# bark-simulator/planner-miqp

Hardware: AMD Instinct MI355X
Metric: MIQP solves/sec to 1% gap, 2-agent x 20-step x 32-region (higher is better)
Workload: dtype f64

## Files before the change

### planner_miqp_amd/csrc/as_onchip.hip

```cpp
namespace miqp {

#ifdef MIQP_PROFILE
#define ASP_T(var) const long long var = clock64()
#define ASP_ACC(k, t0, t1) asp_[k] += (unsigned long long)((t1) - (t0))
#else
#define ASP_T(var)
#define ASP_ACC(k, t0, t1)
#endif
constexpr int AS_MAXSTEP = 220;
constexpr double AS_VTOL = 1.0e-8;
constexpr double AS_DEP = 1.0e-8;
constexpr int AS_MT = 64;
constexpr int AS_MSTR = AS_MT * (AS_MT + 1) / 2;

__host__ __device__ constexpr bool as_shape_ok(int C, int N) { return (C == 1 || C == 2) && N >= 1 && N <= 2 * OC_NSL; }

template <int C> __device__ inline int as_col(int pq) { return C == 2 ? ((pq & 3) << 2) | (pq >> 2) : ((pq & 1) << 2) | (pq >> 1); }
template <int C> __device__ inline int as_pcol(int q) { return C == 2 ? ((q & 3) << 2) | (q >> 2) : ((q & 3) << 1) | (q >> 2); }

template <int C, int NSL, int GCAP = miqp::OC_GCAP>
__global__ void __launch_bounds__(64, (GCAP > 128 ? 1 : 2)) as_onchip_kernel(DevBuf B) {
  static_assert(C == 1 || C == 2, "a stage of 16 columns holds the chains of up to two cars");
  constexpr bool CM = true;
  constexpr bool BIG = GCAP > 128;
  constexpr int OC_GCAP = GCAP, OC_GSLOTS = OC_GCAP / 64, OC_GCOEF = oc_gcoef_of(OC_GCAP);
  constexpr int NX = 6 * C, NZ = 8 * C, NCH = 2 * C;
  const Layout& Y = B.Y;
  const int tid = threadIdx.x, lg = tid >> 4, lc = tid & 15;
  const int par = lg >> 1, side = lg & 1;
  const double bsgn = side ? -1.0 : 1.0;
  WAVE_DUMP(BIG ? 1 : 4);
  const int* const clist = BIG && B.cls_take ? B.cls_list + (size_t)(B.cls_take - 1) * B.batch_cap : nullptr;
  const int nbatch = clist ? (B.cls_count[B.cls_take - 1] < B.batch_cap ? B.cls_count[B.cls_take - 1] : B.batch_cap) : (*B.batch_count < B.batch_cap ? *B.batch_count : B.batch_cap);
  const int N = Y.N, NSLOT = Y.NSLOT;
  extern __shared__ double lds[];
  char* const L0 = (char*)lds;
  const OcLds LL = oc_lds_layout(N, Y.fixlen, OC_GCAP, !BIG);
  double* const Z = (double*)(L0 + LL.z);
  double* const scr = (double*)(L0 + LL.u);
  double* const V = (double*)(L0 + LL.u);
  unsigned long long* const bkey = (unsigned long long*)(L0 + LL.r);
  const int SPAN = LL.gmeta - LL.u;
  double* const kref = (double*)(L0 + LL.u + SPAN - N * 32);
  double* const kff = kref - N * 4;
  double* const KS = kff - N * 16;
  const int STG_CAP = (SPAN - N * 192) / 8;
  uint4* const gmeta = (uint4*)(L0 + LL.gmeta);
  double* const gcoef = (double*)(L0 + LL.gcoef);
  double* const grhs = (double*)(L0 + LL.grhs);
  double* const Wd = (double*)(L0 + LL.wd);
  int* const sstart = (int*)(L0 + LL.sstart);
  unsigned short* const cand = (unsigned short*)(L0 + LL.cand);
// ... 6 lines not shown
  const int chunk = B.as_chunk > 0 ? B.as_chunk : 1;
  int run_next = 0, run_end = 0;
  const int quota = BIG ? 0 : B.as_quota; int handed = 0;
#ifdef MIQP_PROFILE
  const unsigned long long wv_c0 = __builtin_amdgcn_s_memtime(), wv_r0 = __builtin_amdgcn_s_memrealtime();
  unsigned long long wv_first = 0; int wv_nodes = 0;
  if (!BIG && tid == 0) wv_first = atomicMin(&B.prof[120], wv_r0);
#endif
  for (;;) {
    __syncthreads();
    if (run_next >= run_end) {
      if (quota > 0 && handed >= quota) break;
      ++handed;
      if (tid == 0) sh_node = atomicAdd(B.work_counter, chunk);
      __syncthreads();
      run_next = __builtin_amdgcn_readfirstlane(sh_node); run_end = run_next + chunk;
      if (run_next >= nbatch) break;
    }
    const int slot_ = run_next++;
    if (slot_ >= nbatch) { run_next = run_end; continue; }
    const int node = clist ? __builtin_amdgcn_readfirstlane(clist[slot_]) : slot_;
    {
      const int cls = B.batch_large ? (int)B.batch_large[node] : (is_probe_word(B.batch_depth[node]) ? 1 : 0);
      if (cls != (BIG ? 1 : 0)) continue;
    }
    WAVE_DUMP_NODE();
    const int inst = __builtin_amdgcn_readfirstlane(B.batch_inst[node]);
    const double* D = B.inst_d + (size_t)inst * Y.dstride;
    const int* T = B.inst_i + (size_t)inst * Y.istride;
    const double ts = D[Y.d_glob + 7];
    const double aqs = 2.0 * D[Y.d_misc + 0];
    const double iaq = aqs > 0.0 ? 1.0 / aqs : 0.0;
    {
      const signed char* src = B.pool_fix + (size_t)B.batch_node[node] * Y.fixlen;
      for (int k = tid; k < Y.fixlen; k += 64) fix[k] = src[k];
      if (tid < 16) Wd[tid] = tid < NZ ? D[Y.d_wd + oc_lcol<C, CM>(as_pcol<C>(tid))] : 0.0;
      for (int k = tid; k < N * 32; k += 64) bkey[k] = ~0ull;
      for (int k = tid; k <= N + 1; k += 64) sstart[k] = 0;
    }
    __syncthreads();
    const double* Rf = D + Y.d_ref;
    double cutoff = 1e300;
    {
      const double inc0 = fmin(inc_from_key(*(volatile unsigned long long*)&B.inc_key[inst]), B.inc_ext[inst]);
      const double gap_ = is_probe_word(B.batch_depth[node]) ? 0.0 : B.inst_gap[inst];
      if (B.use_cutoff && inc0 < 1e300) cutoff = inc0 - gap_ * (1e-10 + fabs(inc0)) - B.inst_const[inst];
    }

#ifdef MIQP_PROFILE
    unsigned long long asp_[12] = {0, 0, 0, 0, 0, 0, 0, 0, 0, 0, 0, 0};
#endif
    ASP_T(ta0);
    int ngen = 0;
    {
      unsigned long long* const bmp = (unsigned long long*)scr;
      const int nw = (N * NSLOT + 63) >> 6;
      unsigned short* const pre = (unsigned short*)(bmp + nw);
      for (int k = tid; k < nw; k += 64) bmp[k] = 0ull;
      OC_WAVE_SYNC();
      const int cls_off[8] = {0, 7, 11, 16, 16 + Y.EL, 16 + 5 * Y.EL, C * Y.SC, C * Y.SC + 8 * Y.NP};
      const int cls_cnt[8] = {7, 4, 5, Y.EL, 4 * Y.EL, 5 * Y.O, 8 * Y.NP, 16 * Y.NP};
      auto take = [&](int i, int slot) {
        if (decode_row<C, false>(Y, D, T, fix, i, slot, nullptr).active) {
          int col; double sg, rh;
          if (box_of_slot<C>(Y, D, T, fix, i, slot, col, sg, rh)) atomicMin(&bkey[(i * 2 + (sg < 0.0 ? 1 : 0)) * 16 + as_col<C>(oc_pcol<C, CM>(col))], d2key(rh));
          else { const int pcode = i * NSLOT + slot; atomicOr(&bmp[pcode >> 6], 1ull << (pcode & 63)); }
        }
      };
      unsigned short* const plist = pre + ((nw + 1 + 3) & ~3);
      const int LCAP = (int)(((char*)(L0 + LL.r) - (char*)plist) / 2) - 64;
      int nlist = 0;
      auto flush = [&]() {
        OC_WAVE_SYNC();
        for (int j0 = 0; j0 < nlist; j0 += 64) if (j0 + tid < nlist) { const int pc = plist[j0 + tid]; const int i = pc / NSLOT; take(i, pc - i * NSLOT); }
        OC_WAVE_SYNC();
        nlist = 0;
      };
      for (int e0 = 0; e0 < C * N; e0 += 64) {
        const int e = e0 + tid;
        if (e < C * N) {
          const int c = e / N, i = e - c * N;
          const double* G = D + Y.d_glob;
          const int code = i >= 1 ? (int)fix[Y.f_reg + c * N + i] : -1;
          const unsigned int skip = i >= 1 ? (unsigned int)T[Y.i_boxskip + c * N + i] : 0x7Fu;
          const double* rt = code >= 0 ? D + Y.d_reg + (c * Y.P + (code >> 2)) * REGSZ : nullptr;
          const double* Hc = (!rt && i >= 1) ? region_hull(Y, D, T, fix, c, i) : nullptr;
          auto put = [&](int col, bool neg, double rh) { atomicMin(&bkey[(i * 2 + (neg ? 1 : 0)) * 16 + as_col<C>(oc_pcol<C, CM>(col))], d2key(rh)); };
          if (i >= 1) {
            const double a_lo_x = rt ? rt[11] : Hc[0], a_hi_x = rt ? rt[12] : Hc[1], a_lo_y = rt ? rt[13] : Hc[2], a_hi_y = rt ? rt[14] : Hc[3];
            if (!(skip & 1u)) put(6 * c + 1, true, -G[0]);
            if (!(skip & 2u)) put(6 * c + 4, true, -G[0]);
            if (!(skip & 4u)) put(6 * c + 1, false, G[1]);
            if (!(skip & 8u)) put(6 * c + 2, false, a_hi_x);
            if (!(skip & 16u)) put(6 * c + 2, true, -a_lo_x);
            if (!(skip & 32u)) put(6 * c + 5, false, a_hi_y);
            if (!(skip & 64u)) put(6 * c + 5, true, -a_lo_y);
          }
          if (i <= N - 2) {
#pragma unroll
            for (int s_ = 0; s_ < 2; ++s_) {
              double lo, hi;
              if (i == 0) { lo = D[Y.d_u0box + c * 4 + 2 * s_]; hi = D[Y.d_u0box + c * 4 + 2 * s_ + 1]; }
              else if (rt) { lo = rt[15 + 2 * s_]; hi = rt[16 + 2 * s_]; }
              else { lo = Hc[4 + 2 * s_]; hi = Hc[5 + 2 * s_]; }
              put(6 * C + 2 * c + s_, false, hi); put(6 * C + 2 * c + s_, true, -lo);
            }
          }
        }
      }
#pragma unroll 1
      for (int cl = 0; cl < 8; ++cl) {
#ifdef MIQP_PROFILE
        if (cl == 2) { const long long tq_ = clock64(); asp_[9] += (unsigned long long)(tq_ - ta0); }
#endif
        const int cnt = cls_cnt[cl], off = cls_off[cl];
        const bool percar = cl < 6;
        const int per = percar ? C * cnt : cnt, total = N * per;
        for (int e0 = 0; e0 < total; e0 += 64) {
          const int e = e0 + tid;
          int i = 0, slot = 0; bool in = e < total;
          if (in) { i = e / per; const int rem = e - i * per; slot = percar ? (rem / cnt) * Y.SC + off + rem % cnt : off + rem; }
          if (cl < 2) continue;
          const bool cnd = in && slot_maybe<C>(Y, fix, i, slot);
          const unsigned long long mk = __ballot(cnd);
          if (cnd) plist[nlist + __popcll(mk & lt)] = (unsigned short)(i * NSLOT + slot);
          nlist += __popcll(mk);
          if (nlist > LCAP) flush();
        }
      }
      flush();
      if (tid == 0) { int a = 0; for (int k = 0; k < nw; ++k) { pre[k] = (unsigned short)(a < 65535 ? a : 65535); a += __popcll(bmp[k]); } pre[nw] = (unsigned short)(a < 65535 ? a : 65535); }
      OC_WAVE_SYNC();
      ngen = pre[nw];
      if (ngen <= OC_GCAP)
        for (int k = tid; k < nw; k += 64) {
          unsigned long long bits = bmp[k]; int pos = pre[k];
          while (bits) { const int b = __ffsll((long long)bits) - 1; cand[pos++] = (unsigned short)(k * 64 + b); bits &= bits - 1ull; }
        }
      OC_WAVE_SYNC();
    }
#ifdef MIQP_PROFILE
    const long long tq1_ = clock64();
#endif
    bool overflow = ngen > OC_GCAP;
    int ncoef = 0;
    for (int c0 = 0; c0 < ngen && !overflow; c0 += OC_SCR) {
      double* g = scr + (tid & (OC_SCR - 1)) * OC_SSTR;
      RowOut r; r.active = false; r.rhs = 0; r.aq = 0;
      int i = 0, nn = 0;
      const bool mine = tid < OC_SCR && c0 + tid < ngen;
      int slot_ = 0;
      if (mine) { const int pcode = cand[c0 + tid]; i = pcode / NSLOT; slot_ = pcode - i * NSLOT; r = decode_row<C, true>(Y, D, T, fix, i, slot_, g); }
      unsigned long long map = 0ull; unsigned int cols = 0u;
      double v6[6];
#pragma unroll
      for (int k = 0; k < 6; ++k) v6[k] = 0.0;
      if (mine) {
        for (int q = 0; q < NZ; ++q) {
          const double v = g[q];
          if (v != 0.0 && nn < 6) {
#pragma unroll
            for (int k = 0; k < 6; ++k) if (k == nn) v6[k] = v;
            const int pq = as_col<C>(oc_pcol<C, CM>(q));
            map |= (unsigned long long)(nn + 1) << (4 * pq); cols |= (unsigned int)pq << (4 * nn); nn++;
          }
        }
      }
      const bool keep = mine && nn > 0;
      const unsigned long long mk = __ballot(keep);
      const unsigned long long b0 = __ballot(keep && (nn & 1)), b1 = __ballot(keep && (nn & 2)), b2 = __ballot(keep && (nn & 4));
      const int tot = __popcll(b0) + 2 * __popcll(b1) + 4 * __popcll(b2);
      if (ncoef + tot > OC_GCOEF) { overflow = true; break; }
      if (keep) {
        const int idx = sstart[N + 1] + __popcll(mk & lt);
        const int off = ncoef + __popcll(b0 & lt) + 2 * __popcll(b1 & lt) + 4 * __popcll(b2 & lt);
#pragma unroll
        for (int k = 0; k < 6; ++k) if (k < nn) gcoef[off + k] = v6[k];
        uint4 m4; m4.x = (unsigned int)map; m4.y = (unsigned int)(map >> 32);
        m4.z = (unsigned int)off | ((unsigned int)nn << 16) | ((unsigned int)i << 20) | (r.aq > 0.0 ? 0x80000000u : 0u); m4.w = cols;
        gmeta[idx] = m4; grhs[idx] = r.rhs;
        cand[idx] = (unsigned short)(i * NSLOT + slot_);
      }
      OC_WAVE_SYNC();
      if (tid == 0) sstart[N + 1] += __popcll(mk);
      ncoef += tot;
      OC_WAVE_SYNC();
    }
    if (overflow) {
      if (B.batch_A) B.batch_A[(size_t)node * 64 + tid] = 0xFFFFu;
      if (tid == 0) {
        if (B.ring_M) B.batch_Mtag[node] = 0ull;
        B.batch_ok[node] = 5; B.pool_big[B.batch_node[node]] |= (BIG ? 2 : 1); if (B.stats) { atomicAdd(&B.stats[3], 1ull); atomicAdd(&B.stats[8 + (ngen >= 512 ? 15 : ngen / 32)], 1ull); }
      }
      continue;
    }
    const int NM = sstart[N + 1];
    OC_WAVE_SYNC();

    ASP_T(ta1); ASP_ACC(0, ta0, ta1);
#ifdef MIQP_PROFILE
    asp_[11] += (unsigned long long)(ta1 - tq1_);
#endif
    double brhs[NSL];
    unsigned int bact = 0u, binA = 0u, ginA = 0u;
#pragma unroll
    for (int k = 0; k < NSL; ++k) {
      const int i = 2 * k + par;
      brhs[k] = 1e300;
      if (i < N && lc < NZ) {
        const unsigned long long key = bkey[(i * 2 + side) * 16 + lc];
        if (key != ~0ull) { brhs[k] = key2d(key); bact |= 1u << k; }
      }
    }
    OC_WAVE_SYNC();

    const double h1 = ts, h2 = 0.5 * ts * ts, h3 = ts * ts * ts / 6.0;
    const double* const tb = D + Y.d_astab;
    if constexpr (C == 2) {
      for (int k = tid; k < N * 16; k += 64) KS[k] = tb[k];
      for (int k = tid; k < N * 4; k += 64) kref[k] = tb[N * 16 + k];
    } else {
      for (int k = tid; k < N * 8; k += 64) KS[(k >> 3) * 16 + (k & 7)] = tb[k];
      for (int k = tid; k < N * 2; k += 64) kref[(k >> 1) * 4 + (k & 1)] = tb[N * 8 + k];
    }
    OC_WAVE_SYNC();
    typedef double d2_t __attribute__((ext_vector_type(2)));
    auto subst = [&](const bool fromx0, const int itop, const int iend, double* const out) {
      for (int k = tid; k < (N - 1) * 4; k += 64) if ((k >> 2) > itop) kff[k] = fromx0 ? kref[k] : 0.0;
      if (tid < NCH) {
        const int ch = tid;
        double p0 = 0.0, p1 = 0.0, p2 = 0.0;
        int i0 = itop;
        if (itop >= N - 1) { const d2_t a = *(const d2_t*)(V + (N - 1) * 16 + 4 * ch); p0 = a[0]; p1 = a[1]; p2 = V[(N - 1) * 16 + 4 * ch + 2]; i0 = N - 2; }
        if (i0 >= 0) {
          d2_t va = *(const d2_t*)(V + i0 * 16 + 4 * ch), vb = *(const d2_t*)(V + i0 * 16 + 4 * ch + 2);
          d2_t ka = *(const d2_t*)(KS + (i0 * 4 + ch) * 4), kb = *(const d2_t*)(KS + (i0 * 4 + ch) * 4 + 2);
          double kr = fromx0 ? kref[i0 * 4 + ch] : 0.0;
          for (int i = i0; i >= 0; --i) {
            const int j = i > 0 ? i - 1 : 0;
            const d2_t nva = *(const d2_t*)(V + j * 16 + 4 * ch), nvb = *(const d2_t*)(V + j * 16 + 4 * ch + 2);
            const d2_t nka = *(const d2_t*)(KS + (j * 4 + ch) * 4), nkb = *(const d2_t*)(KS + (j * 4 + ch) * 4 + 2);
            const double nkr = fromx0 ? kref[j * 4 + ch] : 0.0;
            const double su = vb[1] + h3 * p0 + h2 * p1 + h1 * p2;
            const double sx0 = va[0] + p0, sx1 = va[1] + h1 * p0 + p1, sx2 = vb[0] + h2 * p0 + h1 * p1 + p2;
            kff[i * 4 + ch] = fma(su, kb[1], kr);
            p0 = sx0 - ka[0] * su; p1 = sx1 - ka[1] * su; p2 = sx2 - kb[0] * su;
            va = nva; vb = nvb; ka = nka; kb = nkb; kr = nkr;
          }
        }
      }
      OC_WAVE_SYNC();
      if (tid < NCH) {
        const int ch = tid;
        double x0 = 0.0, x1 = 0.0, x2 = 0.0;
        if (fromx0) { const int c = ch >> 1, s = ch & 1; x0 = D[Y.d_x0 + 6 * c + 3 * s]; x1 = D[Y.d_x0 + 6 * c + 3 * s + 1]; x2 = D[Y.d_x0 + 6 * c + 3 * s + 2]; }
// ... 360 lines not shown
      lres = fabs(wave_sum(lres));
    } else if (infeas) viol = 1.0;
    if (!fail && !infeas && ok == 1 && !(viol <= 5.0e-7)) { fail = true; why = 5; }
    if (BIG && infeas && B.as_probe_first && B.pump_max > 0 && is_probe_word(B.batch_depth[node]) && (cutoff > 1e299 || B.pump_inc)) fail = true;
    if (fail) {
      if (B.batch_A) B.batch_A[(size_t)node * 64 + tid] = 0xFFFFu;
      if (B.ring_M && tid == 0) B.batch_Mtag[node] = 0ull;
      if (tid == 0) { B.batch_ok[node] = 5; B.pool_big[B.batch_node[node]] |= 4; if (B.as_stats) { sh_stat[2] += 1ull; sh_stat[10 + (why < 6 ? why : 5)] += 1ull; } }
      continue;
    }
    const double obj = (infeas || ok == 2) ? Dval : objective() + scost;
    double* Zo = B.batch_Z + (size_t)node * N * NZ;
    for (int k = tid; k < N * 16; k += 64) { const int q = k & 15; if (q < NZ) Zo[(k >> 4) * NZ + oc_lcol<C, CM>(as_pcol<C>(q))] = Z[k]; }
    if (B.batch_A) {
      unsigned short enc = 0xFFFFu;
      if (!fail && !infeas && ok == 1 && arow >= 0) enc = arow < 1024 ? (unsigned short)arow : (unsigned short)(1024 + (int)cand[arow - 1024]);
      B.batch_A[(size_t)node * 64 + tid] = enc;
    }
    if (B.ring_M) {
      const int n_ = __popcll(used);
      unsigned long long tg_ = 0ull;
      OC_WAVE_SYNC();
      if (!fail && !infeas && ok == 1 && n_ >= 1 && n_ <= AS_MT && n_ * (n_ + 1) * 4 <= LL.total) {
        double* const stg = (double*)L0;
        const int ra = __popcll(used & lt);
#pragma unroll
        for (int b8 = 0; b8 < 64; ++b8) {
          if ((used >> b8) & 1ull) {
            const int rb = __popcll(used & ((1ull << b8) - 1ull));
            if (arow >= 0 && ra >= rb) stg[ra * (ra + 1) / 2 + rb] = M[b8];
          }
        }
        const int len = n_ * (n_ + 1) / 2;
        unsigned long long cnt_ = 0ull;
        if (tid == 0) cnt_ = atomicAdd(B.ring_head, (unsigned long long)len);
        cnt_ = ((unsigned long long)(unsigned int)__builtin_amdgcn_readfirstlane((int)(cnt_ >> 32)) << 32) | (unsigned int)__builtin_amdgcn_readfirstlane((int)cnt_);
        tg_ = (cnt_ << 8) | (unsigned long long)n_;
        OC_WAVE_SYNC();
        const unsigned long long o_ = cnt_ % B.ring_doubles, rd_ = B.ring_doubles;
        for (int k = tid; k < len; k += 64) { unsigned long long q_ = o_ + (unsigned long long)k; if (q_ >= rd_) q_ -= rd_; B.ring_M[q_] = stg[k]; }
      }
      if (tid == 0) B.batch_Mtag[node] = tg_;
    }
    if (tid == 0) {
      B.batch_obj[node] = obj; B.batch_viol[node] = viol; B.batch_ok[node] = ok;
      B.batch_bound[node] = lres + 1e-9 * (1.0 + fabs(obj));
      B.batch_it[node] = steps;
      atomicAdd((unsigned long long*)&B.inst_nodes[inst], 1ull);
      atomicAdd((unsigned long long*)&B.inst_iters[inst], (unsigned long long)steps);
#ifdef MIQP_PROFILE
      ++wv_nodes;
      { const long long tc1 = clock64(); asp_[7] += (unsigned long long)(tc1 - tc0);
        for (int q_ = 0; q_ < 9; ++q_) atomicAdd(&B.prof[80 + q_], asp_[q_]);
        atomicAdd(&B.prof[92], asp_[9]); atomicAdd(&B.prof[93], asp_[11]);
        atomicAdd(&B.prof[90], 1ull); atomicAdd(&B.prof[91], (unsigned long long)steps); }
#endif
      if (B.as_stats) {
        sh_stat[0] += 1ull; sh_stat[1] += (unsigned long long)steps; sh_stat[3] += (unsigned long long)ndrop;
        sh_stat[4] += infeas ? 1ull : 0ull; sh_stat[5] += ok == 2 ? 1ull : 0ull; sh_stat[6] += (unsigned long long)__popcll(used); sh_stat[7] += (unsigned long long)nwarm; sh_stat[8] += (unsigned long long)nfast; sh_stat[9] += (unsigned long long)ncold;
        if (BIG) { const int og_ = B.pool_origin ? (int)B.pool_origin[B.batch_node[node]] : 0; sh_stat[20] += 1ull; sh_stat[21] += (unsigned long long)steps; if (og_ == 14) { sh_stat[22] += 1ull; sh_stat[23] += (unsigned long long)steps; }
          sh_stat[24 + (ngen <= 64 ? 0 : ngen <= 96 ? 1 : ngen <= 128 ? 2 : ngen <= 192 ? 3 : 4)] += 1ull; if (is_probe_word(B.batch_depth[node]) && og_ != 14) sh_stat[29] += 1ull; }
      }
    }
  }
  __syncthreads();
  if (B.as_stats && tid < 32 && sh_stat[tid] != 0ull) atomicAdd(&B.as_stats[tid], sh_stat[tid]);
#ifdef MIQP_PROFILE
  if (!BIG && tid == 0) {
    const unsigned long long wv_c1 = __builtin_amdgcn_s_memtime(), wv_r1 = __builtin_amdgcn_s_memrealtime();
    atomicAdd(&B.prof[94], wv_c1 - wv_c0); atomicAdd(&B.prof[95], wv_r1 - wv_r0); atomicAdd(&B.prof[96], 1ull);
    atomicMin(&B.prof[122], wv_r1); atomicMax(&B.prof[121], wv_r1);
    const unsigned long long dl = wv_r0 > wv_first ? wv_r0 - wv_first : 0ull;
    const int hb = dl < 5000 ? 0 : dl < 20000 ? 1 : dl < 50000 ? 2 : dl < 100000 ? 3 : dl < 200000 ? 4 : dl < 400000 ? 5 : dl < 800000 ? 6 : 7;
    atomicAdd(&B.prof[128 + hb], 1ull);
    const int nb = wv_nodes == 0 ? 0 : wv_nodes <= 4 ? 1 : wv_nodes <= 16 ? 2 : wv_nodes <= 32 ? 3 : wv_nodes <= 64 ? 4 : 5;
    atomicAdd(&B.prof[136 + nb], 1ull);
    if (B.prof[125] == 300 && blockIdx.x < 4096) {
      unsigned int hw, xcc;
      asm volatile("s_getreg_b32 %0, hwreg(HW_REG_HW_ID)" : "=s"(hw));
      asm volatile("s_getreg_b32 %0, hwreg(HW_REG_XCC_ID)" : "=s"(xcc));
      unsigned long long* const w = B.prof + 160 + 4 * blockIdx.x;
      w[0] = wv_r0; w[1] = wv_r1; w[2] = ((unsigned long long)xcc << 32) | hw; w[3] = (unsigned long long)wv_nodes;
    }
  }
#endif
}

}
```

### planner_miqp_amd/csrc/solve_diag.hpp

```cpp
#pragma once

inline void debug_sync(hipStream_t st, int round, const char* stage, int nodes = -1) {
  hipError_t e_ = hipStreamSynchronize(st);
  if (nodes >= 0) std::fprintf(stderr, "[dbg] round %d %s (%d nodes): %s\n", round, stage, nodes, hipGetErrorString(e_));
  else std::fprintf(stderr, "[dbg] round %d %s: %s\n", round, stage, hipGetErrorString(e_));
}

inline bool trace_selection(const DevCtx& X, int rounds, int bc) {
  const DevBuf& B = X.B;
  std::vector<double> sb(bc); std::vector<int> sd(bc); double io_ = 0; int md_ = 0;
  HIP_OK(hipMemcpy(sb.data(), B.batch_bound, (size_t)bc * 8, hipMemcpyDeviceToHost)); HIP_OK(hipMemcpy(sd.data(), B.batch_depth, (size_t)bc * 4, hipMemcpyDeviceToHost));
  HIP_OK(hipMemcpy(&io_, B.inc_obj, 8, hipMemcpyDeviceToHost)); HIP_OK(hipMemcpy(&md_, B.inst_mode, 4, hipMemcpyDeviceToHost));
  std::vector<int> ord(bc); for (int k = 0; k < bc; ++k) ord[k] = k;
  std::sort(ord.begin(), ord.end(), [&](int a, int b) { return sd[a] != sd[b] ? sd[a] > sd[b] : sb[a] < sb[b]; });
  std::fprintf(stderr, "[sel] r%d mode %d incumbent %a:", rounds, md_, io_);
  for (int k : ord) std::fprintf(stderr, " %d.%d/%a", sd[k] >> 6, sd[k] & 63, sb[k]);
  std::fprintf(stderr, "\n");
  return true;
}

inline bool trace_batch(const DevCtx& X, int rounds, int bc) {
  const DevBuf& B = X.B; hipStream_t st = X.stream;
  HIP_OK(hipStreamSynchronize(st));
  if (X.stream2) HIP_OK(hipStreamSynchronize(X.stream2));
// ... 61 lines not shown
#endif
  replay = 0;
  return true;
}

inline bool print_progress(const DevCtx& X, double t, int rounds, long long launched_nodes, double const0) {
  const DevBuf& B = X.B; hipStream_t st = X.stream;
  double lb0 = 0, io0 = 0; int oc0 = 0; unsigned long long k0 = 0;
  HIP_OK(hipMemcpyAsync(&lb0, B.lower_bound, 8, hipMemcpyDeviceToHost, st)); HIP_OK(hipMemcpyAsync(&io0, B.inc_obj, 8, hipMemcpyDeviceToHost, st));
  HIP_OK(hipMemcpyAsync(&oc0, B.open_count, 4, hipMemcpyDeviceToHost, st)); HIP_OK(hipMemcpyAsync(&k0, B.inc_key, 8, hipMemcpyDeviceToHost, st));
  int fc0 = 0; HIP_OK(hipMemcpyAsync(&fc0, B.far_count, 4, hipMemcpyDeviceToHost, st));
  HIP_OK(hipStreamSynchronize(st));
  std::fprintf(stderr, "[miqp_gpu] t %.2f s round %d nodes %lld: instance 0 bound %.4f incumbent %.4f open %d + %d\n", t, rounds, launched_nodes, lb0, k0 >= 0xFFF0000000000000ull ? INFINITY : io0 + const0, oc0, fc0);
  return true;
}

inline bool dump_open_list(const DevCtx& X, const char* dp, int rounds, int NS, double const0) {
  const DevBuf& B = X.B; const Layout& Y = X.Y; const int open_cap = X.open_cap;
  int oc0 = 0; HIP_OK(hipMemcpy(&oc0, B.open_count, 4, hipMemcpyDeviceToHost)); oc0 = std::min(oc0, open_cap);
  const size_t src = ((size_t)(rounds & 1) * NS + 0) * open_cap;
  std::vector<double> hb(oc0); std::vector<int> hn(oc0), hd(oc0);
  if (oc0 > 0) { HIP_OK(hipMemcpy(hb.data(), B.open_bound + src, (size_t)oc0 * 8, hipMemcpyDeviceToHost)); HIP_OK(hipMemcpy(hn.data(), B.open_node + src, (size_t)oc0 * 4, hipMemcpyDeviceToHost));
    HIP_OK(hipMemcpy(hd.data(), B.open_depth + src, (size_t)oc0 * 4, hipMemcpyDeviceToHost)); }
  std::vector<int> ord(oc0); for (int k = 0; k < oc0; ++k) ord[k] = k;
  std::sort(ord.begin(), ord.end(), [&](int x, int y) { return hb[x] < hb[y]; });
  if (FILE* f = std::fopen(dp, "w")) {
    std::fprintf(f, "%d %d %d %d %d %d %d\n", oc0, Y.fixlen, Y.f_reg, Y.f_env, Y.f_obs, Y.f_c2c, Y.N);
    std::vector<signed char> rec(Y.fixlen);
    for (int q = 0; q < std::min(oc0, 400); ++q) {
      int k = ord[q]; HIP_OK(hipMemcpy(rec.data(), B.pool_fix + (size_t)hn[k] * Y.fixlen, Y.fixlen, hipMemcpyDeviceToHost));
      std::fprintf(f, "%.9g %d", hb[k] + const0, hd[k] >> 6); for (int x = 0; x < Y.fixlen; ++x) std::fprintf(f, " %d", (int)rec[x]); std::fprintf(f, "\n");
    }
    std::fclose(f);
  }
  return true;
}

#ifdef MIQP_PROFILE
inline bool print_profile(const DevCtx& X) {
  const DevBuf& B = X.B;
  { unsigned long long pf[64]; HIP_OK(hipMemcpy(pf, B.prof + 64, 64 * 8, hipMemcpyDeviceToHost));
    const char* nm[10] = {"decode", "rowpass", "bw.phi", "bw.TS+p", "bw.readlane+LDL", "bw.Ksolve", "bw.update", "forward", "step", "update"};
    double tot = 0; for (int q = 0; q < 10; ++q) tot += (double)pf[q];
    { unsigned long long po[16]; HIP_OK(hipMemcpy(po, B.prof, 16 * 8, hipMemcpyDeviceToHost));
      const char* no[9] = {"build", "bw.rows/assemble", "bw.mfma", "bw.TS", "bw.cholK", "bw.P", "forward", "step", "update"};
      double to = 0; for (int q = 0; q < 9; ++q) to += (double)po[q];
      if (po[10]) { std::fprintf(stderr, "[miqp_gpu profile] memory-backed kernel nodes %llu iters %llu cycles/node-iter %.0f :", po[10], po[9], to / std::max(1ull, po[9]));
        for (int q = 0; q < 9; ++q) std::fprintf(stderr, " %s %.1f%% (%.0f)", no[q], 100.0 * po[q] / to, (double)po[q] / std::max(1ull, po[9]));
        std::fprintf(stderr, "; inside bw.TS, the stage-Hessian chain: weights + staging %.0f, single-entry rows %.0f, MFMA loop %.0f, reductions + diagonal %.0f", (double)po[12] / std::max(1ull, po[9]), (double)po[13] / std::max(1ull, po[9]), (double)po[14] / std::max(1ull, po[9]), (double)po[15] / std::max(1ull, po[9]));
        std::fprintf(stderr, "\n"); } }
    std::fprintf(stderr, "[miqp_gpu profile] on-chip nodes %llu iters %llu cycles/node-iter %.0f :", pf[11], pf[10], tot / std::max(1ull, pf[10]));
    for (int q = 0; q < 10; ++q) std::fprintf(stderr, " %s %.1f%% (%.0f)", nm[q], 100.0 * pf[q] / tot, (double)pf[q] / std::max(1ull, pf[10]));
    std::fprintf(stderr, "\n");
    { unsigned long long pa[14]; HIP_OK(hipMemcpy(pa, B.prof + 80, 14 * 8, hipMemcpyDeviceToHost));
      const char* na[9] = {"decode", "gains + first iterate", "scan", "response of the row", "q", "directions + ratio test + M update", "iterate refresh", "results", "warm start"};
      double ta = 0; for (int q = 0; q < 9; ++q) ta += (double)pa[q];
      if (pa[10]) { std::fprintf(stderr, "[miqp_gpu profile] active-set kernel nodes %llu steps %llu cycles/node %.0f :", pa[10], pa[11], ta / (double)pa[10]);
        for (int q = 0; q < 9; ++q) std::fprintf(stderr, " %s %.1f%% (%.0f)", na[q], 100.0 * pa[q] / ta, (double)pa[q] / (double)pa[10]);
        std::fprintf(stderr, "; inside the decode: bound classes %.0f, general-row pass %.0f", (double)pa[12] / (double)pa[10], (double)pa[13] / (double)pa[10]);
        std::fprintf(stderr, "\n");
        unsigned long long pw[3], pl[6]; HIP_OK(hipMemcpy(pw, B.prof + 94, 3 * 8, hipMemcpyDeviceToHost)); HIP_OK(hipMemcpy(pl, B.prof + 120, 6 * 8, hipMemcpyDeviceToHost));
        if (pw[2] && pw[1] && pl[5]) std::fprintf(stderr, "[miqp_gpu profile] standard active-set launches: %llu wavefronts resident %.0f shader cycles = %.1f us each (shader clock %.0f MHz); per launch (%llu folded): span %.3f ms, from the first wavefront out of work to the last end %.3f ms, wavefronts %.0f, resident wavefront time / (span x wavefronts) %.3f\n",
          pw[2], (double)pw[0] / pw[2], (double)pw[1] / pw[2] / 100.0, 100.0 * (double)pw[0] / (double)pw[1], pl[5], (double)pl[3] / pl[5] / 1e5, (double)pl[4] / pl[5] / 1e5, (double)pw[2] / pl[5], ((double)pw[1]) / ((double)pl[3] * ((double)pw[2] / pl[5])));
        unsigned long long ph[16]; HIP_OK(hipMemcpy(ph, B.prof + 128, 16 * 8, hipMemcpyDeviceToHost));
        if (pw[2]) { std::fprintf(stderr, "[miqp_gpu profile] standard active-set wavefronts by their start after the launch's first (< 0.05 / 0.2 / 0.5 / 1 / 2 / 4 / 8 ms / later), %% :");
          for (int q = 0; q < 8; ++q) std::fprintf(stderr, " %.1f", 100.0 * ph[q] / pw[2]);
          std::fprintf(stderr, "; by the nodes they solved (0 / <= 4 / <= 16 / <= 32 / <= 64 / more), %% :");
          for (int q = 8; q < 14; ++q) std::fprintf(stderr, " %.1f", 100.0 * ph[q] / pw[2]);
          std::fprintf(stderr, "\n"); }
        if (const char* wd = X.sw.wave_dump) {
          std::vector<unsigned long long> w(4 * 4 * 4096); HIP_OK(hipMemcpy(w.data(), B.prof + 160, w.size() * 8, hipMemcpyDeviceToHost));
          if (FILE* f = std::fopen(wd, "w")) { for (int q = 0; q < 4 * 4096; ++q) if (w[4 * q]) std::fprintf(f, "%d %llu %llu %u %u %llu %d\n", q & 4095, w[4 * q], w[4 * q + 1], (unsigned)(w[4 * q + 2] >> 32), (unsigned)w[4 * q + 2], w[4 * q + 3], q >> 12); std::fclose(f); } } } }
    { unsigned long long pe[8]; HIP_OK(hipMemcpy(pe, B.prof + 100, 8 * 8, hipMemcpyDeviceToHost));
      const char* ne[6] = {"load", "regions", "leaf disjunctions", "branching", "lifting + reservation", "records"};
      double te = 0; for (int q = 0; q < 6; ++q) te += (double)pe[q];
      if (pe[6]) { std::fprintf(stderr, "[miqp_gpu profile] eval_kernel, %llu branched nodes, cycles/node %.0f :", pe[6], te / (double)pe[6]);
        for (int q = 0; q < 6; ++q) std::fprintf(stderr, " %s %.1f%% (%.0f)", ne[q], 100.0 * pe[q] / te, (double)pe[q] / (double)pe[6]);
        std::fprintf(stderr, "\n"); } }
    { unsigned long long ps[10]; HIP_OK(hipMemcpy(ps, B.prof + 110, 10 * 8, hipMemcpyDeviceToHost));
      const char* ns[8] = {"incumbent copy / kill", "setup", "pass 1 (prune, keys)", "far refill", "bound reduce + spill select", "focus + window + share", "radix select + ties", "pass 3 (emit, compact)"};
      double ts = 0; for (int q = 0; q < 8; ++q) ts += (double)ps[q];
      if (ps[8]) { std::fprintf(stderr, "[miqp_gpu profile] select_kernel, %llu workgroups that reached the end (thread 0's clock), mean list %.0f entries, cycles each %.0f :", ps[8], (double)ps[9] / (double)ps[8], ts / (double)ps[8]);
        for (int q = 0; q < 8; ++q) std::fprintf(stderr, " %s %.1f%% (%.0f)", ns[q], 100.0 * ps[q] / ts, (double)ps[q] / (double)ps[8]);
        std::fprintf(stderr, "\n"); } }
    HIP_OK(hipMemset(B.prof, 0, 160 * 8)); }
  return true;
}
#endif

inline bool print_stats(const DevCtx& X) {
  const DevBuf& B = X.B; const Layout& Y = X.Y;
  unsigned long long hs[256]; HIP_OK(hipMemcpy(hs, B.stats, sizeof(hs), hipMemcpyDeviceToHost)); HIP_OK(hipMemset(B.stats, 0, sizeof(hs)));
  const double nn_ = (double)std::max(1ull, hs[0]);
  std::fprintf(stderr, "[miqp_gpu stats] on-chip nodes %llu (general rows %.1f, coefficients %.1f, box keys %.1f, iterations %.1f per node), handed over %llu; general rows / 32 histogram:", hs[0], hs[1] / nn_, hs[4] / nn_, hs[2] / nn_, hs[5] / nn_, hs[3]);
  for (int q = 0; q < 16; ++q) std::fprintf(stderr, " %llu", hs[8 + q]);
  std::fprintf(stderr, "\n");
  std::fprintf(stderr, "[miqp_gpu stats] node outcomes: infeasible %llu (%.1f it), cut off %llu (%.1f it), not converged %llu (%.1f it), solved %llu (%.1f it) of which: bound >= incumbent %llu, within gap %llu, integer feasible %llu, branched %llu (%.2f children; by kind region/env/obstacle/car-car: %llu x %.1f, %llu x %.1f, %llu x %.1f, %llu x %.1f)\n",
               hs[32], hs[36] / (double)std::max(1ull, hs[32]), hs[33], hs[37] / (double)std::max(1ull, hs[33]), hs[34], hs[38] / (double)std::max(1ull, hs[34]), hs[35], hs[39] / (double)std::max(1ull, hs[35]),
               hs[40], hs[41], hs[42], hs[43], hs[44] / (double)std::max(1ull, hs[43]), hs[48], hs[52] / (double)std::max(1ull, hs[48]), hs[49], hs[53] / (double)std::max(1ull, hs[49]),
               hs[50], hs[54] / (double)std::max(1ull, hs[50]), hs[51], hs[55] / (double)std::max(1ull, hs[51]));
  std::fprintf(stderr, "[miqp_gpu stats] region sets: tightened at %llu (car, step) sites, %llu nodes closed because a step had no region left; children not created because of their lifted bound %llu (multi-row lift larger than the single-row one: %llu), car/car sets tightened at %llu groups\n", hs[58], hs[59], hs[56], hs[57], hs[61]);
  std::fprintf(stderr, "[miqp_gpu stats] region branchings flagged by: own rows %llu (worst class acc box %llu, jerk box %llu, sector %llu, half-plane %llu, curvature %llu, slow square %llu), environment front rows %llu, obstacle front rows %llu, car/car front rows %llu; by step:",
               hs[64], hs[70], hs[71], hs[72], hs[73], hs[74], hs[75], hs[65], hs[66], hs[67]);
  for (int q = 0; q < 32 && q < Y.N; ++q) std::fprintf(stderr, " %llu", hs[160 + q]);
  std::fprintf(stderr, "\n[miqp_gpu stats] node outcomes by origin (processed: infeasible / cut off / not converged / solved):");
  const char* on_[16] = {"root|reg-ref", "reg-adjacent", "reg-other", "reg-slow", "env-ref", "env-other", "-", "-", "obs-ref", "obs-other", "-", "-", "c2c-ref", "c2c-other", "-", "probe"};
  for (int q = 0; q < 16; ++q) if (hs[80 + q]) std::fprintf(stderr, " %s %llu: %llu / %llu / %llu / %llu;", on_[q], hs[80 + q], hs[96 + q], hs[112 + q], hs[128 + q], hs[144 + q]);
  std::fprintf(stderr, "\n[miqp_gpu stats] infeasible rounding probes re-rounded: %llu", hs[62]);
  std::fprintf(stderr, "\n[miqp_gpu stats] handed-over nodes with >= 480 general rows: %llu, mean %.0f, most %llu general rows", hs[7], (double)hs[6] / std::max(1ull, hs[7]), hs[5]);
  std::fprintf(stderr, "\n[miqp_gpu stats] rounding probes by iterations / 3 (0-2, 3-5, ..., 45+):");
  { const char* oc_n[4] = {"infeasible", "cut off", "not converged", "solved"};
    for (int o = 0; o < 4; ++o) { std::fprintf(stderr, " %s", oc_n[o]); for (int q = 0; q < 16; ++q) std::fprintf(stderr, " %llu", hs[192 + 16 * o + q]); std::fprintf(stderr, ";"); } }
  std::fprintf(stderr, "\n");
// ... 8 lines not shown
```

Baseline: 1087.

## Replace slot-scan row decode with per-site two-pass decode and wave prefix scan

Replaces the active-set kernel's constraint decode. The old path enumerated candidate slots into a bitmap and list, then decoded each row through a scratch buffer. The new path has each lane own one (step, car-or-pair) site, generate its rows in place, and count them in a first pass. A DPP wave prefix scan then assigns output offsets, and a second pass writes metadata and coefficients directly. This removes the bitmap, list-flush and scratch decode work, at the cost of generating each site's rows twice and uneven lane work when sites differ in row count. The old path stays available behind a compile flag, along with a check mode.

```diff
diff --git a/planner_miqp_amd/csrc/as_decode.hpp b/planner_miqp_amd/csrc/as_decode.hpp
--- /dev/null
+++ b/planner_miqp_amd/csrc/as_decode.hpp
@@ -0,0 +1,206 @@
+#pragma once
+namespace miqp {
+
+__device__ __forceinline__ int as_wave_iscan(int v) {
+  v += __builtin_amdgcn_update_dpp(0, v, 0x111, 0xF, 0xF, true);
+  v += __builtin_amdgcn_update_dpp(0, v, 0x112, 0xF, 0xF, true);
+  v += __builtin_amdgcn_update_dpp(0, v, 0x114, 0xF, 0xF, true);
+  v += __builtin_amdgcn_update_dpp(0, v, 0x118, 0xF, 0xF, true);
+  const int t0 = __builtin_amdgcn_readlane(v, 15), t1 = __builtin_amdgcn_readlane(v, 31), t2 = __builtin_amdgcn_readlane(v, 47);
+  const int r = (int)threadIdx.x >> 4;
+  return v + (r >= 1 ? t0 : 0) + (r >= 2 ? t1 : 0) + (r >= 3 ? t2 : 0);
+}
+
+__device__ __forceinline__ void as_add_point(double (&g)[6], double& rhs, const double* rt, int tx, int ty, double al, double be, const double* K) {
+  g[0] += al;
+  if (tx != PT_R) {
+    if (rt) { const double* p = rt + 19 + (tx == PT_U ? 0 : 3); rhs = __builtin_fma(-al, p[0], rhs); g[1] = __builtin_fma(al, p[1], g[1]); g[4] = __builtin_fma(al, p[2], g[4]); }
+    else if (al != 0.0) rhs = __builtin_fma(-al, K[(tx == PT_U ? 0 : 2) + (al > 0.0 ? 0 : 1)], rhs);
+  }
+  g[3] += be;
+  if (ty != PT_R) {
+    if (rt) { const double* p = rt + 25 + (ty == PT_U ? 0 : 3); rhs = __builtin_fma(-be, p[0], rhs); g[1] = __builtin_fma(be, p[1], g[1]); g[4] = __builtin_fma(be, p[2], g[4]); }
+    else if (be != 0.0) rhs = __builtin_fma(-be, K[(ty == PT_U ? 4 : 6) + (be > 0.0 ? 0 : 1)], rhs);
+  }
+}
+
+struct AsSite {
+  int i, sec;
+  bool on;
+  int code, code2;
+  int dom;
+  const double* rt; const double* rt2;
+  unsigned long long epk, npk;
+};
+
+template <int C>
+__device__ __forceinline__ AsSite as_site_load(const Layout& Y, const double* D, const int* T, const signed char* fix, int site) {
+  constexpr int NPc = C * (C - 1) / 2, U = C + NPc;
+  const int N = Y.N;
+  AsSite S;
+  S.i = site / U; S.sec = site - S.i * U;
+  S.on = S.i >= 1 && S.i < N;
+  S.code = S.code2 = -1; S.dom = 0; S.rt = S.rt2 = nullptr; S.epk = S.npk = 0ull;
+  if (!S.on) return S;
+  const int i = S.i;
+  if (S.sec < C) {
+    const int c = S.sec;
+    S.code = (int)fix[Y.f_reg + c * N + i];
+    if (S.code >= 0) { S.rt = D + Y.d_reg + (c * Y.P + (S.code >> 2)) * REGSZ; S.dom = T[Y.i_dom + (c * Y.P + (S.code >> 2)) * 4 + (S.code & 3)]; }
+    if (Y.E >= 1) {
+      int e[5], ne[5];
+#pragma unroll
+      for (int pt = 0; pt < 5; ++pt) e[pt] = Y.E == 1 ? 0 : (int)fix[Y.f_env + (c * N + i) * 5 + pt];
+#pragma unroll
+      for (int pt = 0; pt < 5; ++pt) ne[pt] = e[pt] >= 0 ? T[Y.i_envn + e[pt]] : 0;
+#pragma unroll
+      for (int pt = 0; pt < 5; ++pt) { S.epk |= (unsigned long long)(unsigned char)e[pt] << (8 * pt); S.npk |= (unsigned long long)(ne[pt] < 0 ? 0 : ne[pt] > 255 ? 255 : ne[pt]) << (8 * pt); }
+    }
+  } else if constexpr (C >= 2) {
+    const int p = S.sec - C;
+    int c1, c2; pair_cars(p, C, c1, c2);
+    S.code = (int)fix[Y.f_reg + c1 * N + i]; S.code2 = (int)fix[Y.f_reg + c2 * N + i];
+    if (S.code >= 0) S.rt = D + Y.d_reg + (c1 * Y.P + (S.code >> 2)) * REGSZ;
+    if (S.code2 >= 0) S.rt2 = D + Y.d_reg + (c2 * Y.P + (S.code2 >> 2)) * REGSZ;
+  }
+  return S;
+}
+
+template <int C, class Box, class Col, class End>
+__device__ __forceinline__ void as_site_rows(const Layout& Y, const double* D, const int* T, const signed char* fix, const AsSite& S, Box&& box, Col&& col, End&& end) {
+  const int N = Y.N, i = S.i;
+  const double* G = D + Y.d_glob;
+  if (S.sec < C) {
+    const int c = S.sec, code = S.code, SC = Y.SC, EL = Y.EL, nenv = Y.E >= 1 ? 5 * EL : 0;
+    const double* const rt = S.rt;
+    int a = 0, b = 0;
+#pragma unroll 1
+    for (int rr = 11; rr < SC; ++rr) {
+      double g[6] = {0.0, 0.0, 0.0, 0.0, 0.0, 0.0};
+      double rhs = 0.0, bsg = 0.0;
+      int kind = 0, bcol = 0;
+      if (rr < 16) {
+        const int k = rr - 11;
+        if (code < 0) {
+          const double* Hc = D + Y.d_hull + (c * N + i) * HULLSZ;
+          if (k <= 1 && Hc[14] != 0.0) { kind = 1; rhs = Hc[10 + 3 * k]; g[1] = Hc[8 + 3 * k]; g[4] = Hc[9 + 3 * k]; }
+        } else {
+          const int h = code & 3;
+          if (h == 3) { if (k <= 3) { kind = 2; bcol = k < 2 ? 1 : 4; bsg = (k & 1) ? -1.0 : 1.0; rhs = G[6]; } }
+          else {
+            kind = 1;
+            switch (k) {
+              case 0: g[1] = rt[0]; g[4] = rt[1]; break;
+              case 1: g[1] = rt[2]; g[4] = rt[3]; break;
+              case 2: {
+                const int* hs = T + Y.i_hs + ((c * Y.P + (code >> 2)) * 2 + h) * 2;
+                kind = 2; bcol = hs[0] == 0 ? 1 : 4; bsg = -(double)hs[1]; rhs = -G[6];
+              } break;
+              case 3: g[5] = 1; g[2] = -rt[4]; g[1] = -rt[6]; g[4] = -rt[7]; rhs = rt[5]; break;
+              default: g[5] = -1; g[2] = rt[4]; g[1] = rt[9]; g[4] = rt[10]; rhs = -rt[8]; break;
+            }
+          }
+        }
+      } else {
+        const bool env = rr < 16 + 5 * EL;
+        const int pt = env ? a : b;
+        const double* ed = nullptr;
+        int tx = PT_R, ty = PT_R;
+        if (env) {
+          const int k = b;
+          if (++b == EL) { b = 0; ++a; }
+          if (rr == 15 + 5 * EL) { a = 0; b = 0; }
+          const int e = (int)(signed char)(unsigned char)(S.epk >> (8 * pt));
+          if (nenv > 0 && e >= 0 && k < (int)((S.npk >> (8 * pt)) & 255ull) && !(pt > 0 && code < 0)) {
+            ed = D + Y.d_env + (e * EL + k) * 3;
+            tx = ENV_PT_D[pt][0]; ty = ENV_PT_D[pt][1];
+            if (pt > 0) {
+              int txs, tys;
+              if (corner_dominated(tx, ty, ed[0], ed[1], S.dom, txs, tys)) {
+                const int ps = env_corner(txs, tys);
+                if ((int)(signed char)(unsigned char)(S.epk >> (8 * ps)) == e) ed = nullptr;
+              }
+            }
+          }
+        } else {
+          const int o = a;
+          if (++b == 5) { b = 0; ++a; }
+          const signed char* fo = fix + Y.f_obs + ((c * Y.O + o) * N + i) * 5;
+          const int kk = (int)fo[pt];
+          if (kk >= 0 && kk < Y.L && !(pt > 0 && code < 0)) {
+            ed = D + Y.d_obs + ((o * N + i) * Y.L + kk) * 3;
+            tx = OBS_PT_D[pt][0]; ty = OBS_PT_D[pt][1];
+            if (pt > 0) {
+              int txs, tys;
+              if (corner_dominated(tx, ty, ed[0], ed[1], S.dom, txs, tys)) {
+                const int ps = obs_corner(txs, tys);
+                if ((int)fo[ps] == kk) ed = nullptr;
+              }
+            }
+          }
+        }
+        if (ed) {
+          const double al = ed[0], be = ed[1];
+          rhs = ed[2];
+          if (pt == 0 && be == 0.0 && fabs(al) == 1.0) { kind = 2; bcol = 0; bsg = al; }
+          else if (pt == 0 && al == 0.0 && fabs(be) == 1.0) { kind = 2; bcol = 3; bsg = be; }
+          else { kind = 1; as_add_point(g, rhs, rt, tx, ty, al, be, nullptr); }
+        }
+      }
+      if (kind == 2) box(6 * c + bcol, bsg < 0.0, rhs);
+      else if (kind == 1) {
+#pragma unroll
+        for (int j = 0; j < 6; ++j) col(g[j], 6 * c + j);
+        end(c * SC + rr, rhs, false);
+      }
+    }
+  } else if constexpr (C >= 2) {
+    const int p = S.sec - C;
+    int c1, c2; pair_cars(p, C, c1, c2);
+    const signed char* const fa = fix + Y.f_c2c + (p * N + i) * 4;
+    const signed char* const fn = fix + Y.f_c2n + (p * N + i) * 4;
+    const double Dsep = D[Y.d_dsep + p * N + i], Ssl = D[Y.d_ssl + i], smax = D[Y.d_smax + i], wsl = D[Y.d_misc + 0];
+    const double* const K1 = (S.code < 0 && !Y.relax_front_off) ? region_fpk(Y, D, T, fix, c1, i) : nullptr;
+    const double* const K2 = (S.code2 < 0 && !Y.relax_front_off) ? region_fpk(Y, D, T, fix, c2, i) : nullptr;
+#pragma unroll 1
+    for (int q = 0; q < 24; ++q) {
+      const bool excl = q >= 8;
+      int grp, which, alt;
+      if (!excl) { grp = q >> 1; which = q & 1; alt = (int)fa[grp]; if (alt < 0) continue; }
+      else { const int q2 = q - 8; grp = q2 >> 2; alt = q2 & 3; which = 1; const int m = (int)fn[grp]; if (m <= 0 || !((m >> alt) & 1)) continue; }
+      const bool need1 = grp >= 2, need2 = (grp == 1 || grp == 3);
+      if (need1 && S.code < 0) { if (excl || Y.relax_front_off || !K1) continue; }
+      if (need2 && S.code2 < 0) { if (excl || Y.relax_front_off || !K2) continue; }
+      const bool soft = (grp == 0 || grp == 3);
+      if (!excl) {
+        if (!soft && which == 1) continue;
+        if (soft && which == 1 && !(smax > 0 && wsl > 0)) continue;
+      }
+      const bool isx = alt < 2, lo = (alt == 0 || alt == 2);
+      int ca, ta, tb;
+      if (grp == 0) { ta = tb = PT_R; ca = lo ? c1 : c2; }
+      else if (grp == 1) { if (lo) { ca = c1; ta = PT_R; tb = PT_L; } else { ca = c2; ta = PT_U; tb = PT_R; } }
+      else if (grp == 2) { if (lo) { ca = c2; ta = PT_R; tb = PT_L; } else { ca = c1; ta = PT_U; tb = PT_R; } }
+      else { if (lo) { ca = c2; ta = PT_U; tb = PT_L; } else { ca = c1; ta = PT_U; tb = PT_L; } }
+      const double al = isx ? 1.0 : 0.0, be = isx ? 0.0 : 1.0;
+      double rhs = soft ? (which == 0 ? -(Dsep + Ssl) + smax : -(Dsep + Ssl)) : -Dsep;
+      const bool sq = !excl && soft && which == 1;
+      const bool a1 = ca == c1;
+      double ga[6] = {0.0, 0.0, 0.0, 0.0, 0.0, 0.0}, gb[6] = {0.0, 0.0, 0.0, 0.0, 0.0, 0.0};
+      as_add_point(ga, rhs, a1 ? S.rt : S.rt2, ta, ta, al, be, a1 ? K1 : K2);
+      as_add_point(gb, rhs, a1 ? S.rt2 : S.rt, tb, tb, -al, -be, a1 ? K2 : K1);
+      if (excl) {
+#pragma unroll
+        for (int k = 0; k < 6; ++k) { ga[k] = -ga[k]; gb[k] = -gb[k]; }
+        rhs = -rhs;
+      }
+#pragma unroll
+      for (int j = 0; j < 6; ++j) col(a1 ? ga[j] : gb[j], 6 * c1 + j);
+#pragma unroll
+      for (int j = 0; j < 6; ++j) col(a1 ? gb[j] : ga[j], 6 * c2 + j);
+      end(C * Y.SC + (excl ? Y.NP * 8 + p * 16 + (q - 8) : p * 8 + q), rhs, sq);
+    }
+  }
+}
+
+}
diff --git a/planner_miqp_amd/csrc/as_onchip.hip b/planner_miqp_amd/csrc/as_onchip.hip
--- a/planner_miqp_amd/csrc/as_onchip.hip
+++ b/planner_miqp_amd/csrc/as_onchip.hip
@@ -1,3 +1,4 @@
+#include "as_decode.hpp"
 namespace miqp {
 
 #ifdef MIQP_PROFILE
@@ -110,6 +111,43 @@
 #endif
     ASP_T(ta0);
     int ngen = 0;
+    bool overflow = false;
+    auto bound_rows = [&](unsigned long long* const bk) {
+      for (int e0 = 0; e0 < C * N; e0 += 64) {
+        const int e = e0 + tid;
+        if (e < C * N) {
+          const int c = e / N, i = e - c * N;
+          const double* G = D + Y.d_glob;
+          const int code = i >= 1 ? (int)fix[Y.f_reg + c * N + i] : -1;
+          const unsigned int skip = i >= 1 ? (unsigned int)T[Y.i_boxskip + c * N + i] : 0x7Fu;
+          const double* rt = code >= 0 ? D + Y.d_reg + (c * Y.P + (code >> 2)) * REGSZ : nullptr;
+          const double* Hc = (!rt && i >= 1) ? region_hull(Y, D, T, fix, c, i) : nullptr;
+          auto put = [&](int col, bool neg, double rh) { atomicMin(&bk[(i * 2 + (neg ? 1 : 0)) * 16 + as_col<C>(oc_pcol<C, CM>(col))], d2key(rh)); };
+          if (i >= 1) {
+            const double a_lo_x = rt ? rt[11] : Hc[0], a_hi_x = rt ? rt[12] : Hc[1], a_lo_y = rt ? rt[13] : Hc[2], a_hi_y = rt ? rt[14] : Hc[3];
+            if (!(skip & 1u)) put(6 * c + 1, true, -G[0]);
+            if (!(skip & 2u)) put(6 * c + 4, true, -G[0]);
+            if (!(skip & 4u)) put(6 * c + 1, false, G[1]);
+            if (!(skip & 8u)) put(6 * c + 2, false, a_hi_x);
+            if (!(skip & 16u)) put(6 * c + 2, true, -a_lo_x);
+            if (!(skip & 32u)) put(6 * c + 5, false, a_hi_y);
+            if (!(skip & 64u)) put(6 * c + 5, true, -a_lo_y);
+          }
+          if (i <= N - 2) {
+#pragma unroll
+            for (int s_ = 0; s_ < 2; ++s_) {
+              double lo, hi;
+              if (i == 0) { lo = D[Y.d_u0box + c * 4 + 2 * s_]; hi = D[Y.d_u0box + c * 4 + 2 * s_ + 1]; }
+              else if (rt) { lo = rt[15 + 2 * s_]; hi = rt[16 + 2 * s_]; }
+              else { lo = Hc[4 + 2 * s_]; hi = Hc[5 + 2 * s_]; }
+              put(6 * C + 2 * c + s_, false, hi); put(6 * C + 2 * c + s_, true, -lo);
+            }
+          }
+        }
+      }
+    };
+#if defined(MIQP_AS_DECODE_OLD) || defined(MIQP_AS_DECODE_CHECK)
+    int ncoef = 0;
     {
       unsigned long long* const bmp = (unsigned long long*)scr;
       const int nw = (N * NSLOT + 63) >> 6;
@@ -134,43 +172,12 @@
         OC_WAVE_SYNC();
         nlist = 0;
       };
-      for (int e0 = 0; e0 < C * N; e0 += 64) {
-        const int e = e0 + tid;
-        if (e < C * N) {
-          const int c = e / N, i = e - c * N;
-          const double* G = D + Y.d_glob;
-          const int code = i >= 1 ? (int)fix[Y.f_reg + c * N + i] : -1;
-          const unsigned int skip = i >= 1 ? (unsigned int)T[Y.i_boxskip + c * N + i] : 0x7Fu;
-          const double* rt = code >= 0 ? D + Y.d_reg + (c * Y.P + (code >> 2)) * REGSZ : nullptr;
-          const double* Hc = (!rt && i >= 1) ? region_hull(Y, D, T, fix, c, i) : nullptr;
-          auto put = [&](int col, bool neg, double rh) { atomicMin(&bkey[(i * 2 + (neg ? 1 : 0)) * 16 + as_col<C>(oc_pcol<C, CM>(col))], d2key(rh)); };
-          if (i >= 1) {
-            const double a_lo_x = rt ? rt[11] : Hc[0], a_hi_x = rt ? rt[12] : Hc[1], a_lo_y = rt ? rt[13] : Hc[2], a_hi_y = rt ? rt[14] : Hc[3];
-            if (!(skip & 1u)) put(6 * c + 1, true, -G[0]);
-            if (!(skip & 2u)) put(6 * c + 4, true, -G[0]);
-            if (!(skip & 4u)) put(6 * c + 1, false, G[1]);
-            if (!(skip & 8u)) put(6 * c + 2, false, a_hi_x);
-            if (!(skip & 16u)) put(6 * c + 2, true, -a_lo_x);
-            if (!(skip & 32u)) put(6 * c + 5, false, a_hi_y);
-            if (!(skip & 64u)) put(6 * c + 5, true, -a_lo_y);
-          }
-          if (i <= N - 2) {
-#pragma unroll
-            for (int s_ = 0; s_ < 2; ++s_) {
-              double lo, hi;
-              if (i == 0) { lo = D[Y.d_u0box + c * 4 + 2 * s_]; hi = D[Y.d_u0box + c * 4 + 2 * s_ + 1]; }
-              else if (rt) { lo = rt[15 + 2 * s_]; hi = rt[16 + 2 * s_]; }
-              else { lo = Hc[4 + 2 * s_]; hi = Hc[5 + 2 * s_]; }
-              put(6 * C + 2 * c + s_, false, hi); put(6 * C + 2 * c + s_, true, -lo);
-            }
-          }
-        }
-      }
+      bound_rows(bkey);
+#ifdef MIQP_PROFILE
+      { const long long tq_ = clock64(); asp_[9] += (unsigned long long)(tq_ - ta0); }
+#endif
 #pragma unroll 1
       for (int cl = 0; cl < 8; ++cl) {
-#ifdef MIQP_PROFILE
-        if (cl == 2) { const long long tq_ = clock64(); asp_[9] += (unsigned long long)(tq_ - ta0); }
-#endif
         const int cnt = cls_cnt[cl], off = cls_off[cl];
         const bool percar = cl < 6;
         const int per = percar ? C * cnt : cnt, total = N * per;
@@ -200,8 +207,7 @@
 #ifdef MIQP_PROFILE
     const long long tq1_ = clock64();
 #endif
-    bool overflow = ngen > OC_GCAP;
-    int ncoef = 0;
+    overflow = ngen > OC_GCAP;
     for (int c0 = 0; c0 < ngen && !overflow; c0 += OC_SCR) {
       double* g = scr + (tid & (OC_SCR - 1)) * OC_SSTR;
       RowOut r; r.active = false; r.rhs = 0; r.aq = 0;
@@ -244,6 +250,93 @@
       ncoef += tot;
       OC_WAVE_SYNC();
     }
+#ifdef MIQP_PROFILE
+    { const long long tq2_ = clock64(); asp_[11] += (unsigned long long)(tq2_ - tq1_); }
+#endif
+#endif
+#ifndef MIQP_AS_DECODE_OLD
+    {
+#ifdef MIQP_AS_DECODE_CHECK
+      const bool o_ovf = overflow; const int o_ngen = ngen, o_nm = sstart[N + 1], o_ncoef = ncoef;
+      unsigned long long* const bk = (unsigned long long*)L0;
+      int bad = 0;
+      OC_WAVE_SYNC();
+      for (int k = tid; k < N * 32; k += 64) bk[k] = ~0ull;
+      OC_WAVE_SYNC();
+#define AS_PUTU(ref, val) do { if ((ref) != (val)) bad = 1; } while (0)
+#define AS_PUTD(ref, val) do { if (__double_as_longlong(ref) != __double_as_longlong(val)) bad = 1; } while (0)
+#else
+      unsigned long long* const bk = bkey;
+#define AS_PUTU(ref, val) (ref) = (val)
+#define AS_PUTD(ref, val) (ref) = (val)
+#endif
+      bound_rows(bk);
+#if defined(MIQP_PROFILE) && !defined(MIQP_AS_DECODE_CHECK)
+      const long long tb_ = clock64(); asp_[9] += (unsigned long long)(tb_ - ta0);
+#endif
+#if defined(MIQP_PROFILE) && !defined(MIQP_AS_DECODE_CHECK)
+      long long tc_ = tb_;
+#endif
+      const AsSite S = as_site_load<C>(Y, D, T, fix, tid);
+      int kbase = 0, cbase = 0, nm_ = 0, ncoef_ = 0;
+#pragma unroll 1
+      for (int ph = 0; ph < 2; ++ph) {
+        int ng_ = 0, nk_ = 0, nc_ = 0, nn = 0;
+        unsigned long long map = 0ull; unsigned int cols = 0u;
+        auto box = [&](int colm, bool neg, double rh) { if (ph == 0) atomicMin(&bk[(S.i * 2 + (neg ? 1 : 0)) * 16 + as_col<C>(oc_pcol<C, CM>(colm))], d2key(rh)); };
+        auto col = [&](double v, int q) {
+          if (v != 0.0 && nn < 6) {
+            if (ph) AS_PUTD(gcoef[cbase + nc_ + nn], v);
+            const int pq = as_col<C>(oc_pcol<C, CM>(q));
+            map |= (unsigned long long)(nn + 1) << (4 * pq); cols |= (unsigned int)pq << (4 * nn); nn++;
+          }
+        };
+        auto end = [&](int slot, double rhs, bool soft) {
+          ++ng_;
+          if (nn > 0) {
+            if (ph) {
+              const int idx = kbase + nk_, off = cbase + nc_;
+              const unsigned int mz = (unsigned int)off | ((unsigned int)nn << 16) | ((unsigned int)S.i << 20) | (soft ? 0x80000000u : 0u);
+              AS_PUTU(gmeta[idx].x, (unsigned int)map); AS_PUTU(gmeta[idx].y, (unsigned int)(map >> 32)); AS_PUTU(gmeta[idx].z, mz); AS_PUTU(gmeta[idx].w, cols);
+              AS_PUTD(grhs[idx], rhs);
+              AS_PUTU(cand[idx], (unsigned short)(S.i * NSLOT + slot));
+            }
+            ++nk_; nc_ += nn;
+          }
+          nn = 0; map = 0ull; cols = 0u;
+        };
+        if (S.on) as_site_rows<C>(Y, D, T, fix, S, box, col, end);
+        if (ph == 0) {
+#if defined(MIQP_PROFILE) && !defined(MIQP_AS_DECODE_CHECK)
+          tc_ = clock64(); asp_[11] += (unsigned long long)(tc_ - tb_);
+#endif
+          const int s1 = as_wave_iscan(ng_ | (nk_ << 16)), s2 = as_wave_iscan(nc_);
+          const int t1 = __builtin_amdgcn_readlane(s1, 63);
+          ngen = t1 & 0xFFFF; nm_ = t1 >> 16; ncoef_ = __builtin_amdgcn_readlane(s2, 63);
+          overflow = ngen > OC_GCAP || ncoef_ > OC_GCOEF;
+          if (overflow) break;
+          kbase = (s1 >> 16) - nk_; cbase = s2 - nc_;
+        }
+      }
+#undef AS_PUTU
+#undef AS_PUTD
+#ifdef MIQP_AS_DECODE_CHECK
+      OC_WAVE_SYNC();
+      for (int k = tid; k < N * 32; k += 64) if (bk[k] != bkey[k]) bad = 1;
+      if (overflow != o_ovf || ngen != o_ngen || (!overflow && (nm_ != o_nm || ncoef_ != o_ncoef))) bad = 1;
+      const unsigned long long anybad = __ballot(bad != 0);
+      if (tid == 0) { atomicAdd(&B.prof[98], 1ull); if (anybad) atomicAdd(&B.prof[99], 1ull); }
+      overflow = o_ovf; ngen = o_ngen;
+      OC_WAVE_SYNC();
+#else
+      if (tid == 0) sstart[N + 1] = nm_;
+      OC_WAVE_SYNC();
+#if defined(MIQP_PROFILE)
+      { const long long tw_ = clock64(); asp_[10] += (unsigned long long)(tw_ - tc_); }
+#endif
+#endif
+    }
+#endif
     if (overflow) {
       if (B.batch_A) B.batch_A[(size_t)node * 64 + tid] = 0xFFFFu;
       if (tid == 0) {
@@ -256,9 +349,6 @@
     OC_WAVE_SYNC();
 
     ASP_T(ta1); ASP_ACC(0, ta0, ta1);
-#ifdef MIQP_PROFILE
-    asp_[11] += (unsigned long long)(ta1 - tq1_);
-#endif
     double brhs[NSL];
     unsigned int bact = 0u, binA = 0u, ginA = 0u;
 #pragma unroll
@@ -725,7 +815,7 @@
       ++wv_nodes;
       { const long long tc1 = clock64(); asp_[7] += (unsigned long long)(tc1 - tc0);
         for (int q_ = 0; q_ < 9; ++q_) atomicAdd(&B.prof[80 + q_], asp_[q_]);
-        atomicAdd(&B.prof[92], asp_[9]); atomicAdd(&B.prof[93], asp_[11]);
+        atomicAdd(&B.prof[92], asp_[9]); atomicAdd(&B.prof[93], asp_[11]); atomicAdd(&B.prof[97], asp_[10]);
         atomicAdd(&B.prof[90], 1ull); atomicAdd(&B.prof[91], (unsigned long long)steps); }
 #endif
       if (B.as_stats) {
diff --git a/planner_miqp_amd/csrc/solve_diag.hpp b/planner_miqp_amd/csrc/solve_diag.hpp
--- a/planner_miqp_amd/csrc/solve_diag.hpp
+++ b/planner_miqp_amd/csrc/solve_diag.hpp
@@ -137,13 +137,21 @@
     std::fprintf(stderr, "[miqp_gpu profile] on-chip nodes %llu iters %llu cycles/node-iter %.0f :", pf[11], pf[10], tot / std::max(1ull, pf[10]));
     for (int q = 0; q < 10; ++q) std::fprintf(stderr, " %s %.1f%% (%.0f)", nm[q], 100.0 * pf[q] / tot, (double)pf[q] / std::max(1ull, pf[10]));
     std::fprintf(stderr, "\n");
-    { unsigned long long pa[14]; HIP_OK(hipMemcpy(pa, B.prof + 80, 14 * 8, hipMemcpyDeviceToHost));
+    { unsigned long long pa[20]; HIP_OK(hipMemcpy(pa, B.prof + 80, 20 * 8, hipMemcpyDeviceToHost));
       const char* na[9] = {"decode", "gains + first iterate", "scan", "response of the row", "q", "directions + ratio test + M update", "iterate refresh", "results", "warm start"};
       double ta = 0; for (int q = 0; q < 9; ++q) ta += (double)pa[q];
       if (pa[10]) { std::fprintf(stderr, "[miqp_gpu profile] active-set kernel nodes %llu steps %llu cycles/node %.0f :", pa[10], pa[11], ta / (double)pa[10]);
         for (int q = 0; q < 9; ++q) std::fprintf(stderr, " %s %.1f%% (%.0f)", na[q], 100.0 * pa[q] / ta, (double)pa[q] / (double)pa[10]);
-        std::fprintf(stderr, "; inside the decode: bound classes %.0f, general-row pass %.0f", (double)pa[12] / (double)pa[10], (double)pa[13] / (double)pa[10]);
+#if defined(MIQP_AS_DECODE_OLD) || defined(MIQP_AS_DECODE_CHECK)
+        std::fprintf(stderr, "; inside the decode: bound classes %.0f, general-row pass %.0f, rest %.0f", (double)pa[12] / (double)pa[10], (double)pa[13] / (double)pa[10], ((double)pa[0] - (double)pa[12] - (double)pa[13]) / (double)pa[10]);
+#else
+        std::fprintf(stderr, "; inside the decode: bound classes %.0f, site pass (count) %.0f, scan + write %.0f, rest %.0f", (double)pa[12] / (double)pa[10], (double)pa[13] / (double)pa[10], (double)pa[17] / (double)pa[10],
+                     ((double)pa[0] - (double)pa[12] - (double)pa[13] - (double)pa[17]) / (double)pa[10]);
+#endif
         std::fprintf(stderr, "\n");
+#ifdef MIQP_AS_DECODE_CHECK
+        std::fprintf(stderr, "[miqp_gpu profile] decode check: nodes %llu mismatching %llu\n", pa[18], pa[19]);
+#endif
         unsigned long long pw[3], pl[6]; HIP_OK(hipMemcpy(pw, B.prof + 94, 3 * 8, hipMemcpyDeviceToHost)); HIP_OK(hipMemcpy(pl, B.prof + 120, 6 * 8, hipMemcpyDeviceToHost));
         if (pw[2] && pw[1] && pl[5]) std::fprintf(stderr, "[miqp_gpu profile] standard active-set launches: %llu wavefronts resident %.0f shader cycles = %.1f us each (shader clock %.0f MHz); per launch (%llu folded): span %.3f ms, from the first wavefront out of work to the last end %.3f ms, wavefronts %.0f, resident wavefront time / (span x wavefronts) %.3f\n",
           pw[2], (double)pw[0] / pw[2], (double)pw[1] / pw[2] / 100.0, 100.0 * (double)pw[0] / (double)pw[1], pl[5], (double)pl[3] / pl[5] / 1e5, (double)pl[4] / pl[5] / 1e5, (double)pw[2] / pl[5], ((double)pw[1]) / ((double)pl[3] * ((double)pw[2] / pl[5])));
```

Measured after the change: 1066, median of 2. 0.98x the previous value.
